# PytorchConnectomics/pytorch_connectomics

Measured on AMD Instinct MI355X. Metric: voxels/s (train + sliding-window infer), MedNeXt-S 112^3 bf16, higher is better.
Workload: dtype bf16; 1 GPU; Lucchi++ sliding-window inference (configs[1]): MedNeXt-S k3, 165x1024x768 volume, roi 112^3, overlap 0.5, bump blending, sw_batch_size 8, random-init weights; step = one whole-volume EagerSlidingWindowEngine call (TTA off); value = window-voxels/s; sw_batch_size=8, window_pipeline_streams=3

## Files before the change

### pytorch_connectomics_amd/csrc/build.py

```python
from __future__ import annotations

import hashlib
import os
import subprocess
import sys
from concurrent.futures import ThreadPoolExecutor
from pathlib import Path

CSRC = Path(__file__).resolve().parent
PKG = CSRC.parent
LIB_DIR = PKG / "lib"
LIB = LIB_DIR / "libpytc_hip.so"
ARCH = "gfx950"
FLAGS = ["-O3", "-std=c++17", "-fPIC", f"--offload-arch={ARCH}", "-Wno-unused-result"]


_NO_SLP = os.environ.get("PYTC_NO_SLP_FILES", "dwconv_kernels.hip,dwconv_mfma_kernels.hip,train_kernels.hip,rsunet_train_kernels.hip,"
                         "conv3d_strided_kernels.hip,loss_optim_kernels.hip,volume_kernels.hip,upcat_kernels.hip")
EXTRA_FLAGS = {p.name: ["-fno-slp-vectorize"] for p in Path(__file__).resolve().parent.glob("*.hip")
               if _NO_SLP == "all" or p.name in _NO_SLP.split(",")}

NO_SPILL_KERNELS = {"dwconv_kernels.hip": ("dwconv3d_k3_march_kernel", "dw_wgrad_march_kernel"),
                    "dwconv_mfma_kernels.hip": ("dwconv3d_k3_mfma_kernel",)}


def _check_no_spills(fname: str, remarks: str, patterns) -> None:
    import re
    name = None
    for line in remarks.splitlines():
        m = re.search(r"Function Name: (\S+)", line)
        if m:
            name = m.group(1)
            continue
        m = re.search(r"(VGPRs Spill|ScratchSize \[bytes/lane\]): (\d+)", line)
        if m and name and any(p in name for p in patterns) and int(m.group(2)) != 0:
            raise RuntimeError(f"{fname}: kernel {name} reports {m.group(1)} = {m.group(2)}; the asm-load / counted-wait kernels "
                               "must be spill-free (lower the occupancy hint of that instantiation)")


def asm_listing(src: Path, hipcc: str = "/opt/rocm/bin/hipcc") -> str:
    import tempfile
    with tempfile.TemporaryDirectory() as td:
        out = Path(td) / (src.stem + ".s")
        subprocess.run([hipcc, *FLAGS, *EXTRA_FLAGS.get(src.name, []), "-S", "--cuda-device-only", str(src), "-o", str(out)],
                       check=True, capture_output=True)
        return out.read_text()


def _check_asm_load_discipline(src: Path, hipcc: str) -> None:
    from . import asm_check
    text = asm_listing(src, hipcc)
    pats = NO_SPILL_KERNELS[src.name]
    if asm_check.asm_loads_in(text, pats) == 0:
        raise RuntimeError(f"{src.name}: no asm-issued register loads found in kernels {pats}: the ISA check would be checking nothing")
    bad = asm_check.check_listing(text, pats)
    if bad:
        raise RuntimeError(f"{src.name}: {len(bad)} violations of the asm-load discipline (csrc/asm_check.py), e.g.\n  " + "\n  ".join(bad[:5]))


def _check_packed_fp32_selects(obj: Path) -> None:
    import re
    objdump = Path(os.environ.get("HIPCC", "/opt/rocm/bin/hipcc")).resolve().parent.parent / "lib" / "llvm" / "bin" / "llvm-objdump"
    if not objdump.exists():
        objdump = Path("/opt/rocm/lib/llvm/bin/llvm-objdump")
    if not objdump.exists():
        return
    subprocess.run([str(objdump), "--offloading", obj.name], cwd=obj.parent, check=True, capture_output=True)
    pat = re.compile(r"v_pk_(fma|mul|add)_f32 .*op_sel:\[")
    try:
        for co in obj.parent.glob(obj.name + ".*gfx950*"):
            dis = subprocess.run([str(objdump), "-d", str(co)], check=True, capture_output=True, text=True).stdout
            hits = [ln.strip() for ln in dis.splitlines() if pat.search(ln)]
            if hits:
                raise RuntimeError(f"{obj.name}: {len(hits)} packed-fp32 instructions with a low-lane high-dword select, e.g. "
                                   f"`{hits[0]}`; add the source to PYTC_NO_SLP_FILES / EXTRA_FLAGS in csrc/build.py")
    finally:
        for extra in obj.parent.glob(obj.name + ".*"):
            extra.unlink()


def _sources():
    return sorted(CSRC.glob("*.hip"))


def _digest() -> str:
    h = hashlib.sha256()
    for p in _sources() + sorted(CSRC.glob("*.h")) + [PKG.parent / "include" / "pytc_hip.h"]:
        h.update(p.name.encode())
        h.update(p.read_bytes())
    h.update(" ".join(FLAGS).encode())
    h.update(repr(sorted(EXTRA_FLAGS.items())).encode())
    return h.hexdigest()


def build(force: bool = False, verbose: bool = True) -> Path:
    LIB_DIR.mkdir(exist_ok=True)
    obj_dir = LIB_DIR / "obj"
    obj_dir.mkdir(exist_ok=True)
    stamp = LIB_DIR / "build.sha256"
    dig = _digest()
    if not force and LIB.exists() and stamp.exists() and stamp.read_text().strip() == dig:
        build_h5(verbose=verbose)
        return LIB
    hipcc = os.environ.get("HIPCC", "/opt/rocm/bin/hipcc")

    headers = sorted(CSRC.glob("*.h")) + [PKG.parent / "include" / "pytc_hip.h", Path(__file__), CSRC / "asm_check.py"]

    def object_digest(src: Path) -> str:
        h = hashlib.sha256()
        for q in [src] + headers:
            h.update(q.name.encode())
            h.update(q.read_bytes())
        h.update(" ".join(FLAGS + EXTRA_FLAGS.get(src.name, [])).encode())
        return h.hexdigest()

    def compile_one(src: Path) -> Path:
        obj = obj_dir / (src.stem + ".o")
        ostamp = obj_dir / (src.stem + ".sha256")
        odig = object_digest(src)
        if not force and obj.exists() and ostamp.exists() and ostamp.read_text().strip() == odig:
            return obj
        cmd = [hipcc, *FLAGS, *EXTRA_FLAGS.get(src.name, []), "-c", str(src), "-o", str(obj)]
        if verbose:
            print("[build]", " ".join(cmd), flush=True)
        if src.name in NO_SPILL_KERNELS:
            out = subprocess.run(cmd + ["-Rpass-analysis=kernel-resource-usage"], check=True, capture_output=True, text=True).stderr
            _check_no_spills(src.name, out, NO_SPILL_KERNELS[src.name])
            _check_asm_load_discipline(src, hipcc)
        else:
            subprocess.run(cmd, check=True)
        _check_packed_fp32_selects(obj)
        ostamp.write_text(odig)
        return obj

    with ThreadPoolExecutor(max_workers=min(8, os.cpu_count() or 1)) as ex:
        objs = list(ex.map(compile_one, _sources()))
    cmd = [hipcc, "-shared", "-fPIC", f"--offload-arch={ARCH}", *map(str, objs), "-o", str(LIB)]
    if verbose:
        print("[build]", " ".join(cmd), flush=True)
    subprocess.run(cmd, check=True)
    stamp.write_text(dig)
    build_h5(verbose=verbose)
    return LIB


H5_LIB = LIB_DIR / "libpytc_h5.so"
H5_SRC = CSRC / "host" / "h5io.c"


def build_h5(verbose: bool = True):
    for root in (os.environ.get("HDF5_ROOT"), "/opt/conda", "/usr"):
        if root and (Path(root) / "include" / "hdf5.h").exists() and list((Path(root) / "lib").glob("libhdf5.so*")):
            break
    else:
        if verbose:
            print("[build] HDF5 headers not found: libpytc_h5.so skipped")
        return None
    if H5_LIB.exists() and H5_LIB.stat().st_mtime >= H5_SRC.stat().st_mtime:
        return H5_LIB
    LIB_DIR.mkdir(exist_ok=True)
    cmd = ["gcc", "-O2", "-fPIC", "-shared", f"-I{root}/include", str(H5_SRC), f"-L{root}/lib", "-lhdf5", "-lz", "-lpthread", "-ldl",
           f"-Wl,-rpath,{root}/lib", "-o", str(H5_LIB)]
    if verbose:
        print("[build]", " ".join(cmd), flush=True)
    subprocess.run(cmd, check=True)
    return H5_LIB


if __name__ == "__main__":
    print(build(force="--force" in sys.argv))
```

### pytorch_connectomics_amd/csrc/dwconv_mfma_kernels.hip

```cpp
#include <type_traits>

#include "dwconv_march.h"
#include "pw_common.h"

namespace pytc {

typedef short s4_t __attribute__((ext_vector_type(4)));
typedef unsigned int u32x4_t __attribute__((ext_vector_type(4)));
typedef unsigned int u32x2a4_t __attribute__((ext_vector_type(2), aligned(4)));
typedef __bf16 bf2_t __attribute__((ext_vector_type(2)));
typedef float f2_t __attribute__((ext_vector_type(2)));

constexpr int MF_TY = 8, MF_TX = 8, MF_CG = 32;
constexpr int MF_EY = MF_TY + 2, MF_EX = MF_TX + 2;
constexpr int MF_EXP = 16;
constexpr int MF_CS = MF_EY * MF_EXP + 2;
constexpr int MF_IMG = MF_CG * MF_CS;
constexpr int MF_NCHUNK = MF_EY * MF_EX * (MF_CG / 8);
constexpr int MF_CPT = 2;
constexpr int MF_TS = 32;
constexpr int MF_RS = MF_TX * MF_TS + 8;

__device__ __forceinline__ unsigned short mf_bf16_bits(float f) {
  unsigned int u = __float_as_uint(f);
  u += 0x7FFFu + ((u >> 16) & 1u);
  return (unsigned short)(u >> 16);
}
__device__ __forceinline__ float mf_bf16_float(unsigned short h) { return __uint_as_float(((unsigned int)h) << 16); }

template <int N>
__device__ __forceinline__ void mf_wait_vm() { asm volatile("s_waitcnt vmcnt(%0)" : : "n"(N) : "memory"); }


template <int N>
__device__ __forceinline__ void mf_wait_vm_upto(int n) {
  if constexpr (N > 0) {
    if (n >= N) { mf_wait_vm<N>(); return; }
    mf_wait_vm_upto<N - 1>(n);
  } else {
    mf_wait_vm<0>();
  }
}

template <int PF, bool LO, int PROBE = 0, bool STORE = true, int MIXHC = 0>
__global__ void __launch_bounds__(256, MIXHC ? 3 : 4)
dwconv3d_k3_mfma_kernel(const unsigned short* __restrict__ x, unsigned short* __restrict__ y, const float* __restrict__ w,
                        const float* __restrict__ bias, float* __restrict__ stats, DwMarch g, DwMix mx) {
  static_assert(PF == 2 || PF == 3, "two or three planes in flight");
  static_assert(MIXHC == 0 || (STORE && PF == 3), "the fused block keeps the output tile and three planes in flight");
  constexpr bool MIX = MIXHC > 0;
  __shared__ __attribute__((aligned(16))) bf16x8_t w2s[MIX ? MIXHC * 2 * 64 : 1];
  __shared__ __attribute__((aligned(16))) h8_t w3s[MIX ? 2 * MIXHC * 64 : 1];
  __shared__ __attribute__((aligned(16))) float mbias[MIX ? 32 * MIXHC + 32 : 4];
  __shared__ __attribute__((aligned(16))) unsigned short image[2][MF_IMG];
  __shared__ __attribute__((aligned(16))) unsigned short otile[STORE ? 2 : 1][STORE ? MF_TY * MF_RS : 8];
  __shared__ float wl[27 * MF_CG];
  __shared__ float red[4][2][16];

  const int tid = threadIdx.x, wave = tid >> 6, lane = tid & 63;
  int b = g.swizzle ? xcd_swizzle(blockIdx.x, gridDim.x) : blockIdx.x;
  const int ncg = g.C / MF_CG;
  const int cg = g.cg_inner ? b % ncg : (b / g.slots) % ncg;
  const int slot_id = g.cg_inner ? (b / ncg) % g.slots : b % g.slots;
  const int n = b / (ncg * g.slots);
  b = slot_id;
  const int fx = b % g.tx; b /= g.tx;
  const int fy = b % g.ty;
  const int zchunk = b / g.ty;
  const int y0 = fy * MF_TY, x0 = fx * MF_TX;
  const int zs = zchunk * g.zc;
  const int ze = min(zs + g.zc, g.D);
  const int C = g.C;
  const long plane_elems = (long)g.H * g.W * C;
  const unsigned short* xn = x + (long)n * g.D * plane_elems + cg * MF_CG;
  unsigned short* yn = y + (long)n * g.D * plane_elems + cg * MF_CG;
  const bool inner = y0 >= 1 && y0 + MF_TY + 1 <= g.H && x0 >= 1 && x0 + MF_TX + 1 <= g.W;

  for (int i = tid; i < 27 * MF_CG; i += 256) wl[i] = w[(long)(i / MF_CG) * C + cg * MF_CG + (i % MF_CG)];
  if constexpr (MIX) {
    const bf16x8_t* w2g = mx.w2n + (long)n * mx.w2_stride;
    for (int i = tid; i < MIXHC * 2 * 64; i += 256) { w2s[i] = w2g[i]; w3s[i] = mx.w3[i]; }
    if (tid < 32 * MIXHC) mbias[tid] = mx.b2n[(long)n * (32 * MIXHC) + tid];
    else if (tid < 32 * MIXHC + 32) mbias[tid] = mx.b3[tid - 32 * MIXHC];
  }
  __syncthreads();

  int goff[MF_CPT], loff[MF_CPT];
  bool cok[MF_CPT];
#pragma unroll
  for (int i = 0; i < MF_CPT; ++i) {
    const int c = tid + 256 * i;
    const int vox = c >> 2, part = c & 3;
    const int yy = vox / MF_EX, xx = vox % MF_EX;
    const int gy = y0 - 1 + yy, gx = x0 - 1 + xx;
    cok[i] = (c < MF_NCHUNK) && gy >= 0 && gy < g.H && gx >= 0 && gx < g.W;
    const int gyc = min(max(gy, 0), g.H - 1), gxc = min(max(gx, 0), g.W - 1);
    goff[i] = (gyc * g.W + gxc) * C + part * 8;
    loff[i] = (c < MF_NCHUNK) ? (part * 8) * MF_CS + yy * MF_EXP + xx : -1;
  }
  u32x4_t stg[PF][MF_CPT];
  auto issue = [&](int gz, u32x4_t (&st)[MF_CPT]) {
    const int zc = min(max(gz, 0), g.D - 1);
#pragma unroll
    for (int i = 0; i < MF_CPT; ++i) {
      const unsigned short* ptr = xn + (long)zc * plane_elems + goff[i];
      asm volatile("global_load_dwordx4 %0, %1, off" : "=&v"(st[i]) : "v"(ptr) : "memory");
    }
  };
  auto landed = [&](u32x4_t (&st)[MF_CPT], int younger) {
    mf_wait_vm_upto<2 * MF_CPT + 2>(younger);
    asm volatile("" : "+v"(st[0]), "+v"(st[1]) : : "memory");
  };
  auto commit = [&](int slot, u32x4_t (&st)[MF_CPT], int gz) {
    const bool zok = gz >= 0 && gz < g.D;
#pragma unroll
    for (int i = 0; i < MF_CPT; ++i) {
      if (loff[i] < 0) continue;
      unsigned short* dst = &image[slot][loff[i]];
      if (inner && zok) {
#pragma unroll
        for (int q = 0; q < 4; ++q) {
          dst[(2 * q) * MF_CS] = (unsigned short)(st[i][q] & 0xffffu);
          dst[(2 * q + 1) * MF_CS] = (unsigned short)(st[i][q] >> 16);
        }
      } else {
        const bool ok = zok && cok[i];
#pragma unroll
        for (int q = 0; q < 4; ++q) {
          const unsigned int dw = ok ? st[i][q] : 0u;
          dst[(2 * q) * MF_CS] = (unsigned short)(dw & 0xffffu);
          dst[(2 * q + 1) * MF_CS] = (unsigned short)(dw >> 16);
        }
      }
    }
  };

  const int h = wave & 1, ph = wave >> 1;
  const int cl = lane >> 2, j = lane & 3;
  const int ch = h * 16 + cl;
  s4_t a_hi[3][2], a_lo[3][2];
#pragma unroll
  for (int dy = 0; dy < 3; ++dy)
#pragma unroll
    for (int r = 0; r < 2; ++r) {
      s4_t vh, vl;
#pragma unroll
      for (int k = 0; k < 4; ++k) {
        const int i = j;
        const int dz = 2 - i, dx = k - r;
        float wv = 0.f;
        if (i < 3 && dx >= 0 && dx < 3) wv = wl[((dz * 3 + dy) * 3 + dx) * MF_CG + ch];
        const unsigned short hb = mf_bf16_bits(wv);
        vh[k] = (short)hb;
        vl[k] = (short)mf_bf16_bits(wv - mf_bf16_float(hb));
      }
      a_hi[dy][r] = vh;
      a_lo[dy][r] = vl;
    }
  float bv = bias ? bias[cg * MF_CG + ch] : 0.f;
  asm volatile("" : "+v"(bv));

  int boff[4];
  bool pok[4][2];
#pragma unroll
  for (int u = 0; u < 4; ++u) {
    boff[u] = ch * MF_CS + (ph * 4 + j) * MF_EXP + 2 * u;
#pragma unroll
    for (int r = 0; r < 2; ++r) pok[u][r] = (y0 + ph * 4 + j) < g.H && (x0 + 2 * u + r) < g.W;
  }
  const int op = tid >> 2, opiece = tid & 3;
  const int oy = op >> 3, ox = op & 7;
  const bool ook = (y0 + oy) < g.H && (x0 + ox) < g.W;
  const long obase = ((long)(y0 + oy) * g.W + (x0 + ox)) * C + opiece * 8;
  const int orb = oy * MF_RS + ox * MF_TS + opiece * 8;
  int ooff[4];
#pragma unroll
  for (int u = 0; u < 4; ++u) ooff[u] = (ph * 4 + j) * MF_RS + (2 * u) * MF_TS + ch;
  auto flush = [&](int zo) {
    const u32x4_t o = *reinterpret_cast<const u32x4_t*>(&otile[zo & 1][orb]);
    if (ook) *reinterpret_cast<u32x4_t*>(yn + (long)zo * plane_elems + obase) = o;
  };

  const int mr = lane & 15, mkb = lane >> 4;
  const int mp = wave * 16 + mr, my = mp >> 3, mxx = mp & 7;
  const bool mok = (y0 + my) < g.H && (x0 + mxx) < g.W;
  const long mbase = ((long)min(y0 + my, g.H - 1) * g.W + min(x0 + mxx, g.W - 1)) * C + mkb * 8;
  const int mtile = my * MF_RS + mxx * MF_TS + mkb * 8;
  u32x4_t rres[MIX ? 3 : 1];
  auto issue_res = [&](int z, u32x4_t& rr) {
    const unsigned short* ptr = xn + (long)z * plane_elems + mbase;
    asm volatile("global_load_dwordx4 %0, %1, off" : "=&v"(rr) : "v"(ptr) : "memory");
  };
  auto mix = [&](int zo, u32x4_t& rr, int younger) {
    if constexpr (MIX) {
      const bf16x8_t bact = *reinterpret_cast<const bf16x8_t*>(&otile[zo & 1][mtile]);
      f32x4_t acc2[2] = {*reinterpret_cast<const f32x4_t*>(&mbias[32 * MIXHC + mkb * 8]), *reinterpret_cast<const f32x4_t*>(&mbias[32 * MIXHC + mkb * 8 + 4])};
#pragma unroll
      for (int hc = 0; hc < MIXHC; ++hc) {
        f32x4_t acc1[2] = {*reinterpret_cast<const f32x4_t*>(&mbias[hc * 32 + mkb * 8]), *reinterpret_cast<const f32x4_t*>(&mbias[hc * 32 + mkb * 8 + 4])};
#pragma unroll
        for (int mt = 0; mt < 2; ++mt) acc1[mt] = Mma<bf16_t>::mma(w2s[(hc * 2 + mt) * 64 + lane], bact, acc1[mt]);
        float gg[8];
#pragma unroll
        for (int q = 0; q < 4; ++q) { gg[q] = acc1[0][q]; gg[4 + q] = acc1[1][q]; }
        const h8_t bhh = gelu_h8_from_f32(gg);
#pragma unroll
        for (int mo = 0; mo < 2; ++mo) acc2[mo] = __builtin_amdgcn_mfma_f32_16x16x32_f16(w3s[(mo * MIXHC + hc) * 64 + lane], bhh, acc2[mo], 0, 0, 0);
      }
      float v[8];
#pragma unroll
      for (int q = 0; q < 4; ++q) { v[q] = acc2[0][q]; v[4 + q] = acc2[1][q]; }
      if (mx.residual) {
        mf_wait_vm_upto<5>(younger);
        asm volatile("" : "+v"(rr) : : "memory");
        float rv[8];
        VecIO<bf16_t, 8>::load(reinterpret_cast<const bf16_t*>(&rr), rv);
#pragma unroll
        for (int q = 0; q < 8; ++q) v[q] += rv[q];
      }
      const long vo = (long)zo * plane_elems + mbase;
      if (mx.head_w) {
        const bf16x8_t ob = Mma<bf16_t>::from_floats(v);
        if (mx.store_y && mok) *reinterpret_cast<bf16x8_t*>(yn + vo) = ob;
        const f32x4_t hh = Mma<bf16_t>::mma(mx.head_w[lane], ob, f32x4_t{0.f, 0.f, 0.f, 0.f});
        if (mok) {
          float* hy = mx.head_y + ((long)n * g.D * g.H * g.W + (vo - mkb * 8) / C) * mx.n_head;
#pragma unroll
          for (int i = 0; i < 4; ++i)
            if (mkb * 4 + i < mx.n_head) hy[mkb * 4 + i] = hh[i] + (mx.head_b ? mx.head_b[mkb * 4 + i] : 0.f);
        }
      } else if (mok) {
        VecIO<bf16_t, 8>::store(reinterpret_cast<bf16_t*>(yn + vo), v);
      }
    }
  };

  f32x4_t acc[4][2];
#pragma unroll
  for (int u = 0; u < 4; ++u)
#pragma unroll
    for (int r = 0; r < 2; ++r) acc[u][r] = f32x4_t{bv, bv, bv, 0.f};
  float s1 = 0.f, s2 = 0.f;
  unsigned long long tk[9] = {0, 0, 0, 0, 0, 0, 0, 0, 0}, tlast = 0, tstart = 0;
  auto stamp = [&](int k) {
    if constexpr (PROBE == 4) {
      const unsigned long long now = __builtin_amdgcn_s_memtime();
      tk[k] += now - tlast;
      tlast = now;
    }
  };
  if constexpr (PROBE == 4) { tstart = __builtin_amdgcn_s_memtime(); tlast = tstart; }

  auto exists_p = [&](int z) { return z <= ze; };
  auto exists_r = [&](int z) { return MIX && mx.residual && z >= zs && z < ze; };
  auto step = [&](int gz, int slot, u32x4_t (&ld)[MF_CPT], u32x4_t (&cm)[MF_CPT], u32x4_t& rn, u32x4_t& ro) {
    if constexpr (MIX) {
      if (gz - 2 >= zs) mix(gz - 2, ro, (exists_p(gz + 1) ? MF_CPT : 0) + (exists_r(gz - 1) ? 1 : 0) + (exists_p(gz + 2) ? MF_CPT : 0));
      stamp(8);
      if (exists_r(gz)) issue_res(gz, rn);
    } else {
      if (STORE && gz - 2 >= zs && PROBE != 3) flush(gz - 2);
    }
    if (gz + PF <= ze) issue(gz + PF, ld);
    stamp(0);
    const unsigned short* img = image[slot];
#pragma unroll
    for (int dy = 0; dy < ((PROBE == 1 || PROBE == 3) ? 0 : 3); ++dy) {
      s4_t bq[4];
#pragma unroll
      for (int u = 0; u < 4; ++u) bq[u] = __builtin_bit_cast(s4_t, *reinterpret_cast<const u32x2a4_t*>(img + boff[u] + dy * MF_EXP));
#pragma unroll
      for (int u = 0; u < 4; ++u)
#pragma unroll
        for (int r = 0; r < 2; ++r) acc[u][r] = __builtin_amdgcn_mfma_f32_4x4x4bf16_1k(a_hi[dy][r], bq[u], acc[u][r], 0, 0, 0);
      if (LO) {
#pragma unroll
        for (int u = 0; u < 4; ++u)
#pragma unroll
          for (int r = 0; r < 2; ++r) acc[u][r] = __builtin_amdgcn_mfma_f32_4x4x4bf16_1k(a_lo[dy][r], bq[u], acc[u][r], 0, 0, 0);
      }
    }
    stamp(1);
    if (gz + 1 <= ze) {
      landed(cm, MF_CPT * min(PF - 1, ze - gz - 1) + (exists_r(gz - 1) ? 1 : 0) + (exists_r(gz) ? 1 : 0));
      stamp(2);
      commit(slot ^ 1, cm, gz + 1);
      stamp(3);
    } else {
      mf_wait_vm<0>();
    }
    if (gz - 1 >= zs && PROBE != 3) {
      unsigned short* ot = otile[STORE ? (gz - 1) & 1 : 0];
#pragma unroll
      for (int u = 0; u < 4; ++u) {
        const bf2_t hb = __builtin_convertvector(f2_t{acc[u][0][0], acc[u][1][0]}, bf2_t);
        const unsigned int bits = __builtin_bit_cast(unsigned int, hb);
        if constexpr (STORE) {
          ot[ooff[u]] = (unsigned short)(bits & 0xffffu);
          ot[ooff[u] + MF_TS] = (unsigned short)(bits >> 16);
        }
        if constexpr (!MIX) {
          float r0 = __uint_as_float(bits << 16), r1 = __uint_as_float(bits & 0xffff0000u);
          if (!inner) { r0 = pok[u][0] ? r0 : 0.f; r1 = pok[u][1] ? r1 : 0.f; }
          s1 += r0; s2 = fmaf(r0, r0, s2);
          s1 += r1; s2 = fmaf(r1, r1, s2);
        }
      }
    }
#pragma unroll
    for (int u = 0; u < 4; ++u)
#pragma unroll
      for (int r = 0; r < 2; ++r) acc[u][r] = f32x4_t{acc[u][r][1], acc[u][r][2], bv, 0.f};
    stamp(4);
    __syncthreads();
    stamp(5);
    if constexpr (PROBE == 4) tk[6] += 1;
  };

#pragma unroll
  for (int q = 0; q < PF; ++q) issue(zs - 1 + q, stg[q]);
  landed(stg[0], MF_CPT * (PF - 1));
  commit(0, stg[0], zs - 1);
  __syncthreads();
  int slot = 0;
  for (int gz = zs - 1; gz <= ze; gz += PF) {
#pragma unroll
    for (int k = 0; k < PF; ++k) {
      if (gz + k <= ze) { step(gz + k, slot, stg[k], stg[(k + 1) % PF], rres[MIX ? k : 0], rres[MIX ? (k + 1) % 3 : 0]); slot ^= 1; }
    }
  }
  mf_wait_vm<0>();
  if constexpr (MIX) {
    const int rs = (ze - zs) % 3;
    if (rs == 0) mix(ze - 1, rres[0], 0);
    else if (rs == 1) mix(ze - 1, rres[MIX ? 1 : 0], 0);
    else mix(ze - 1, rres[MIX ? 2 : 0], 0);
  } else {
    if (STORE && PROBE != 3) flush(ze - 1);
  }

  if constexpr (PROBE == 4) {
    if constexpr (MIX) {
      if (mx.prof && lane == 0) {
        tk[7] = __builtin_amdgcn_s_memtime() - tstart;
        float* o = mx.prof + (((long)n * g.slots + slot_id) * 4 + wave) * 9;
#pragma unroll
        for (int k = 0; k < 9; ++k) o[k] = (float)tk[k];
      }
    } else if (stats && lane == 0) {
      tk[7] = __builtin_amdgcn_s_memtime() - tstart;
      float* o = stats + (((long)n * g.slots + slot_id) * 2) * C + cg * MF_CG + wave * 8;
#pragma unroll
      for (int k = 0; k < 8; ++k) o[k] = (float)tk[k];
    }
    return;
  }
  if (!MIX && stats) {
    s1 += __shfl_xor(s1, 1, 64); s2 += __shfl_xor(s2, 1, 64);
    s1 += __shfl_xor(s1, 2, 64); s2 += __shfl_xor(s2, 2, 64);
    if (j == 0) { red[wave][0][cl] = s1; red[wave][1][cl] = s2; }
    __syncthreads();
    if (tid < 2 * MF_CG) {
      const int which = tid / MF_CG, chn = tid % MF_CG;
      const float a = red[chn >> 4][which][chn & 15] + red[(chn >> 4) + 2][which][chn & 15];
      stats[(((long)n * g.slots + slot_id) * 2 + which) * C + cg * MF_CG + chn] = a;
    }
  }
}

void dwconv_mfma_launch(const void* x, void* y, const float* w, const float* bias, float* stats, const DwMarch& g, int variant,
                        hipStream_t s) {
  dim3 grid((unsigned)((long)g.slots * (g.C / MF_CG) * g.N)), block(256);
  const unsigned short* xp = (const unsigned short*)x;
  unsigned short* yp = (unsigned short*)y;
  const DwMix none{};
#define PYTC_MF(PFV, LOV, NM) hipLaunchKernelGGL((dwconv3d_k3_mfma_kernel<PFV, LOV, NM>), grid, block, 0, s, xp, yp, w, bias, stats, g, none)
#define PYTC_MF_STATS(PFV, LOV) hipLaunchKernelGGL((dwconv3d_k3_mfma_kernel<PFV, LOV, 0, false>), grid, block, 0, s, xp, yp, w, bias, stats, g, none)
  const int probe = tuning_get("dwconv_mfma_probe", 0);
  if (!y) {
    if (variant & 1) { if (variant & 2) PYTC_MF_STATS(2, true); else PYTC_MF_STATS(3, true); }
    else { if (variant & 2) PYTC_MF_STATS(2, false); else PYTC_MF_STATS(3, false); }
  }
  else if (probe == 1) PYTC_MF(3, false, 1);
  else if (probe == 3) PYTC_MF(3, false, 3);
  else if (probe == 4) PYTC_MF(3, false, 4);
  else if (variant & 1) { if (variant & 2) PYTC_MF(2, true, 0); else PYTC_MF(3, true, 0); }
  else { if (variant & 2) PYTC_MF(2, false, 0); else PYTC_MF(3, false, 0); }
#undef PYTC_MF
#undef PYTC_MF_STATS
}

int dwmix_launch(const void* x, void* y, const float* w, const float* bias, const DwMarch& g, const DwMix& mx, int c_hid, int variant,
                 hipStream_t s) {
  dim3 grid((unsigned)((long)g.slots * g.N)), block(256);
  const unsigned short* xp = (const unsigned short*)x;
  unsigned short* yp = (unsigned short*)y;
#define PYTC_DM(LOV, HCV, PRB) hipLaunchKernelGGL((dwconv3d_k3_mfma_kernel<3, LOV, PRB, true, HCV>), grid, block, 0, s, xp, yp, w, bias, (float*)nullptr, g, mx)
  const bool lo = variant & 1;
  if (mx.prof) {
    if (c_hid != 64 || lo) return -1;
    PYTC_DM(false, 2, 4);
    return 0;
  }
  switch (c_hid) {
    case 64: if (lo) PYTC_DM(true, 2, 0); else PYTC_DM(false, 2, 0); break;
    case 96: if (lo) PYTC_DM(true, 3, 0); else PYTC_DM(false, 3, 0); break;
    case 128: if (lo) PYTC_DM(true, 4, 0); else PYTC_DM(false, 4, 0); break;
    default: return -1;
  }
#undef PYTC_DM
  return 0;
}

}
```

Measured before the change: 1.820 billion voxels/s.

## Add warp-specialized fused dwconv+MLP kernel with separate conv and mix waves

Adds a 512-thread kernel where four waves run the depthwise 3x3x3 MFMA march and four other waves run the pointwise expand/GELU/project mix (plus residual and optional head) on the previous plane via a double-buffered LDS output tile. It becomes the default path for the fused dwmix launch through an env/tuning switch. The intent is to overlap the depthwise convolution and the channel-mixing matmuls instead of running them serially in one set of waves. The cost is more LDS per block, 2 blocks per CU rather than 3, and barrier coupling between the two wave groups.

```diff
diff --git a/pytorch_connectomics_amd/csrc/build.py b/pytorch_connectomics_amd/csrc/build.py
--- a/pytorch_connectomics_amd/csrc/build.py
+++ b/pytorch_connectomics_amd/csrc/build.py
@@ -21,7 +21,7 @@
                if _NO_SLP == "all" or p.name in _NO_SLP.split(",")}
 
 NO_SPILL_KERNELS = {"dwconv_kernels.hip": ("dwconv3d_k3_march_kernel", "dw_wgrad_march_kernel"),
-                    "dwconv_mfma_kernels.hip": ("dwconv3d_k3_mfma_kernel",)}
+                    "dwconv_mfma_kernels.hip": ("dwconv3d_k3_mfma_kernel", "dwmix_waves_kernel")}
 
 
 def _check_no_spills(fname: str, remarks: str, patterns) -> None:
diff --git a/pytorch_connectomics_amd/csrc/dwconv_mfma_kernels.hip b/pytorch_connectomics_amd/csrc/dwconv_mfma_kernels.hip
--- a/pytorch_connectomics_amd/csrc/dwconv_mfma_kernels.hip
+++ b/pytorch_connectomics_amd/csrc/dwconv_mfma_kernels.hip
@@ -1,3 +1,5 @@
+#include <stdlib.h>
+
 #include <type_traits>
 
 #include "dwconv_march.h"
@@ -31,6 +33,8 @@
 template <int N>
 __device__ __forceinline__ void mf_wait_vm() { asm volatile("s_waitcnt vmcnt(%0)" : : "n"(N) : "memory"); }
 
+
+__device__ __forceinline__ void mf_lds_barrier() { asm volatile("s_waitcnt lgkmcnt(0)\n\ts_barrier" : : : "memory"); }
 
 template <int N>
 __device__ __forceinline__ void mf_wait_vm_upto(int n) {
@@ -368,6 +372,273 @@
   }
 }
 
+template <bool LO, int MIXHC>
+__global__ void __launch_bounds__(512, 2)
+dwmix_waves_kernel(const unsigned short* __restrict__ x, unsigned short* __restrict__ y, const float* __restrict__ w,
+                   const float* __restrict__ bias, DwMarch g, DwMix mx) {
+  constexpr int PF = 3;
+  __shared__ __attribute__((aligned(16))) bf16x8_t w2s[MIXHC * 2 * 64];
+  __shared__ __attribute__((aligned(16))) h8_t w3s[2 * MIXHC * 64];
+  __shared__ __attribute__((aligned(16))) float mbias[32 * MIXHC + 32];
+  __shared__ __attribute__((aligned(16))) unsigned short image[2][MF_IMG];
+  __shared__ __attribute__((aligned(16))) unsigned short otile[2][MF_TY * MF_RS];
+  __shared__ float wl[27 * MF_CG];
+
+  const int tid = threadIdx.x, lane = tid & 63;
+  const int wave = __builtin_amdgcn_readfirstlane(tid >> 6);
+  int b = g.swizzle ? xcd_swizzle(blockIdx.x, gridDim.x) : blockIdx.x;
+  const int slot_id = b % g.slots;
+  const int n = b / g.slots;
+  b = slot_id;
+  const int fx = b % g.tx; b /= g.tx;
+  const int fy = b % g.ty;
+  const int zchunk = b / g.ty;
+  const int y0 = fy * MF_TY, x0 = fx * MF_TX;
+  const int zs = zchunk * g.zc;
+  const int ze = min(zs + g.zc, g.D);
+  const int C = MF_CG;
+  const long plane_elems = (long)g.H * g.W * C;
+  const unsigned short* xn = x + (long)n * g.D * plane_elems;
+  unsigned short* yn = y + (long)n * g.D * plane_elems;
+
+  for (int i = tid; i < 27 * MF_CG; i += 512) wl[i] = w[i];
+  {
+    const bf16x8_t* w2g = mx.w2n + (long)n * mx.w2_stride;
+    for (int i = tid; i < MIXHC * 2 * 64; i += 512) { w2s[i] = w2g[i]; w3s[i] = mx.w3[i]; }
+    if (tid < 32 * MIXHC) mbias[tid] = mx.b2n[(long)n * (32 * MIXHC) + tid];
+    else if (tid < 32 * MIXHC + 32) mbias[tid] = mx.b3[tid - 32 * MIXHC];
+  }
+  __syncthreads();
+
+  if (wave < 4) {
+    const bool inner = y0 >= 1 && y0 + MF_TY + 1 <= g.H && x0 >= 1 && x0 + MF_TX + 1 <= g.W;
+    int goff[MF_CPT], loff[MF_CPT];
+    bool cok[MF_CPT];
+#pragma unroll
+    for (int i = 0; i < MF_CPT; ++i) {
+      const int c = tid + 256 * i;
+      const int vox = c >> 2, part = c & 3;
+      const int yy = vox / MF_EX, xx = vox % MF_EX;
+      const int gy = y0 - 1 + yy, gx = x0 - 1 + xx;
+      cok[i] = (c < MF_NCHUNK) && gy >= 0 && gy < g.H && gx >= 0 && gx < g.W;
+      const int gyc = min(max(gy, 0), g.H - 1), gxc = min(max(gx, 0), g.W - 1);
+      goff[i] = (gyc * g.W + gxc) * C + part * 8;
+      loff[i] = (c < MF_NCHUNK) ? (part * 8) * MF_CS + yy * MF_EXP + xx : -1;
+    }
+    u32x4_t stg[PF][MF_CPT];
+    auto issue = [&](int gz, u32x4_t (&st)[MF_CPT]) {
+      const int zc = min(max(gz, 0), g.D - 1);
+#pragma unroll
+      for (int i = 0; i < MF_CPT; ++i) {
+        const unsigned short* ptr = xn + (long)zc * plane_elems + goff[i];
+        asm volatile("global_load_dwordx4 %0, %1, off" : "=&v"(st[i]) : "v"(ptr) : "memory");
+      }
+    };
+    auto landed = [&](u32x4_t (&st)[MF_CPT], int younger) {
+      mf_wait_vm_upto<2 * MF_CPT>(younger);
+      asm volatile("" : "+v"(st[0]), "+v"(st[1]) : : "memory");
+    };
+    auto commit = [&](int slot, u32x4_t (&st)[MF_CPT], int gz) {
+      const bool zok = gz >= 0 && gz < g.D;
+#pragma unroll
+      for (int i = 0; i < MF_CPT; ++i) {
+        if (loff[i] < 0) continue;
+        unsigned short* dst = &image[slot][loff[i]];
+        if (inner && zok) {
+#pragma unroll
+          for (int q = 0; q < 4; ++q) {
+            dst[(2 * q) * MF_CS] = (unsigned short)(st[i][q] & 0xffffu);
+            dst[(2 * q + 1) * MF_CS] = (unsigned short)(st[i][q] >> 16);
+          }
+        } else {
+          const bool ok = zok && cok[i];
+#pragma unroll
+          for (int q = 0; q < 4; ++q) {
+            const unsigned int dw = ok ? st[i][q] : 0u;
+            dst[(2 * q) * MF_CS] = (unsigned short)(dw & 0xffffu);
+            dst[(2 * q + 1) * MF_CS] = (unsigned short)(dw >> 16);
+          }
+        }
+      }
+    };
+
+    const int h = wave & 1, ph = wave >> 1;
+    const int cl = lane >> 2, j = lane & 3;
+    const int ch = h * 16 + cl;
+    s4_t a_hi[3][2], a_lo[3][2];
+#pragma unroll
+    for (int dy = 0; dy < 3; ++dy)
+#pragma unroll
+      for (int r = 0; r < 2; ++r) {
+        s4_t vh, vl;
+#pragma unroll
+        for (int k = 0; k < 4; ++k) {
+          const int i = j;
+          const int dz = 2 - i, dx = k - r;
+          float wv = 0.f;
+          if (i < 3 && dx >= 0 && dx < 3) wv = wl[((dz * 3 + dy) * 3 + dx) * MF_CG + ch];
+          const unsigned short hb = mf_bf16_bits(wv);
+          vh[k] = (short)hb;
+          vl[k] = (short)mf_bf16_bits(wv - mf_bf16_float(hb));
+        }
+        a_hi[dy][r] = vh;
+        a_lo[dy][r] = vl;
+      }
+    float bv = bias ? bias[ch] : 0.f;
+    asm volatile("" : "+v"(bv));
+
+    int boff[4], ooff[4];
+#pragma unroll
+    for (int u = 0; u < 4; ++u) {
+      boff[u] = ch * MF_CS + (ph * 4 + j) * MF_EXP + 2 * u;
+      ooff[u] = (ph * 4 + j) * MF_RS + (2 * u) * MF_TS + ch;
+    }
+    f32x4_t acc[4][2];
+#pragma unroll
+    for (int u = 0; u < 4; ++u)
+#pragma unroll
+      for (int r = 0; r < 2; ++r) acc[u][r] = f32x4_t{bv, bv, bv, 0.f};
+
+    auto step = [&](int gz, int slot, u32x4_t (&ld)[MF_CPT], u32x4_t (&cm)[MF_CPT]) {
+      if (gz + PF <= ze) issue(gz + PF, ld);
+      const unsigned short* img = image[slot];
+#pragma unroll
+      for (int dy = 0; dy < 3; ++dy) {
+        s4_t bq[4];
+#pragma unroll
+        for (int u = 0; u < 4; ++u) bq[u] = __builtin_bit_cast(s4_t, *reinterpret_cast<const u32x2a4_t*>(img + boff[u] + dy * MF_EXP));
+#pragma unroll
+        for (int u = 0; u < 4; ++u)
+#pragma unroll
+          for (int r = 0; r < 2; ++r) acc[u][r] = __builtin_amdgcn_mfma_f32_4x4x4bf16_1k(a_hi[dy][r], bq[u], acc[u][r], 0, 0, 0);
+        if (LO) {
+#pragma unroll
+          for (int u = 0; u < 4; ++u)
+#pragma unroll
+            for (int r = 0; r < 2; ++r) acc[u][r] = __builtin_amdgcn_mfma_f32_4x4x4bf16_1k(a_lo[dy][r], bq[u], acc[u][r], 0, 0, 0);
+        }
+      }
+      if (gz + 1 <= ze) {
+        landed(cm, MF_CPT * min(PF - 1, ze - gz - 1));
+        commit(slot ^ 1, cm, gz + 1);
+      } else {
+        mf_wait_vm<0>();
+      }
+      if (gz - 1 >= zs) {
+        unsigned short* ot = otile[(gz - 1) & 1];
+#pragma unroll
+        for (int u = 0; u < 4; ++u) {
+          const bf2_t hb = __builtin_convertvector(f2_t{acc[u][0][0], acc[u][1][0]}, bf2_t);
+          const unsigned int bits = __builtin_bit_cast(unsigned int, hb);
+          ot[ooff[u]] = (unsigned short)(bits & 0xffffu);
+          ot[ooff[u] + MF_TS] = (unsigned short)(bits >> 16);
+        }
+      }
+#pragma unroll
+      for (int u = 0; u < 4; ++u)
+#pragma unroll
+        for (int r = 0; r < 2; ++r) acc[u][r] = f32x4_t{acc[u][r][1], acc[u][r][2], bv, 0.f};
+      __syncthreads();
+    };
+
+#pragma unroll
+    for (int q = 0; q < PF; ++q) issue(zs - 1 + q, stg[q]);
+    landed(stg[0], MF_CPT * (PF - 1));
+    commit(0, stg[0], zs - 1);
+    __syncthreads();
+    int slot = 0;
+    for (int gz = zs - 1; gz <= ze; gz += PF) {
+#pragma unroll
+      for (int k = 0; k < PF; ++k) {
+        if (gz + k <= ze) { step(gz + k, slot, stg[k], stg[(k + 1) % PF]); slot ^= 1; }
+      }
+    }
+    mf_wait_vm<0>();
+  } else {
+    const int mr = lane & 15, mkb = lane >> 4;
+    const int mp = (wave - 4) * 16 + mr, my = mp >> 3, mxx = mp & 7;
+    const bool mok = (y0 + my) < g.H && (x0 + mxx) < g.W;
+    const long mbase = ((long)min(y0 + my, g.H - 1) * g.W + min(x0 + mxx, g.W - 1)) * C + mkb * 8;
+    const int mtile = my * MF_RS + mxx * MF_TS + mkb * 8;
+    bf16x8_t hw{};
+    float hb[4] = {0.f, 0.f, 0.f, 0.f};
+    if (mx.head_w) {
+      hw = mx.head_w[lane];
+#pragma unroll
+      for (int i = 0; i < 4; ++i)
+        if (mx.head_b && mkb * 4 + i < mx.n_head) hb[i] = mx.head_b[mkb * 4 + i];
+    }
+    auto issue_res = [&](int z, u32x4_t& rr) {
+      const unsigned short* ptr = xn + (long)z * plane_elems + mbase;
+      asm volatile("global_load_dwordx4 %0, %1, off" : "=&v"(rr) : "v"(ptr) : "memory");
+    };
+    auto mix = [&](int zo, u32x4_t& rr, int younger, auto res_tag) {
+      constexpr bool RES = decltype(res_tag)::value;
+      const bf16x8_t bact = *reinterpret_cast<const bf16x8_t*>(&otile[zo & 1][mtile]);
+      f32x4_t acc2[2] = {*reinterpret_cast<const f32x4_t*>(&mbias[32 * MIXHC + mkb * 8]), *reinterpret_cast<const f32x4_t*>(&mbias[32 * MIXHC + mkb * 8 + 4])};
+#pragma unroll
+      for (int hc = 0; hc < MIXHC; ++hc) {
+        f32x4_t acc1[2] = {*reinterpret_cast<const f32x4_t*>(&mbias[hc * 32 + mkb * 8]), *reinterpret_cast<const f32x4_t*>(&mbias[hc * 32 + mkb * 8 + 4])};
+#pragma unroll
+        for (int mt = 0; mt < 2; ++mt) acc1[mt] = Mma<bf16_t>::mma(w2s[(hc * 2 + mt) * 64 + lane], bact, acc1[mt]);
+        float gg[8];
+#pragma unroll
+        for (int q = 0; q < 4; ++q) { gg[q] = acc1[0][q]; gg[4 + q] = acc1[1][q]; }
+        const h8_t bhh = gelu_h8_from_f32(gg);
+#pragma unroll
+        for (int mo = 0; mo < 2; ++mo) acc2[mo] = __builtin_amdgcn_mfma_f32_16x16x32_f16(w3s[(mo * MIXHC + hc) * 64 + lane], bhh, acc2[mo], 0, 0, 0);
+      }
+      float v[8];
+#pragma unroll
+      for (int q = 0; q < 4; ++q) { v[q] = acc2[0][q]; v[4 + q] = acc2[1][q]; }
+      if constexpr (RES) {
+        mf_wait_vm_upto<1>(younger);
+        asm volatile("" : "+v"(rr) : : "memory");
+        float rv[8];
+        VecIO<bf16_t, 8>::load(reinterpret_cast<const bf16_t*>(&rr), rv);
+#pragma unroll
+        for (int q = 0; q < 8; ++q) v[q] += rv[q];
+      }
+      const long vo = (long)zo * plane_elems + mbase;
+      if (mx.head_w) {
+        const bf16x8_t ob = Mma<bf16_t>::from_floats(v);
+        if (mx.store_y && mok) *reinterpret_cast<bf16x8_t*>(yn + vo) = ob;
+        const f32x4_t hh = Mma<bf16_t>::mma(hw, ob, f32x4_t{0.f, 0.f, 0.f, 0.f});
+        if (mok) {
+          float* hy = mx.head_y + ((long)n * g.D * g.H * g.W + (vo - mkb * 8) / C) * mx.n_head;
+#pragma unroll
+          for (int i = 0; i < 4; ++i)
+            if (mkb * 4 + i < mx.n_head) hy[mkb * 4 + i] = hh[i] + hb[i];
+        }
+      } else if (mok) {
+        VecIO<bf16_t, 8>::store(reinterpret_cast<bf16_t*>(yn + vo), v);
+      }
+    };
+    auto march = [&](auto res_tag) {
+      constexpr bool RES = decltype(res_tag)::value;
+      u32x4_t rres[2] = {u32x4_t{0u, 0u, 0u, 0u}, u32x4_t{0u, 0u, 0u, 0u}};
+      mf_lds_barrier();
+      for (int gz0 = zs - 1; gz0 <= ze; gz0 += 2) {
+#pragma unroll
+        for (int k = 0; k < 2; ++k) {
+          const int gz = gz0 + k;
+          if (gz <= ze) {
+            if (gz - 2 >= zs) mix(gz - 2, rres[k], gz - 1 < ze ? 1 : 0, res_tag);
+            else if (RES) mf_wait_vm<1>();
+            if (RES && gz >= zs && gz < ze) issue_res(gz, rres[k]);
+            mf_lds_barrier();
+          }
+        }
+      }
+      mf_wait_vm<0>();
+      u32x4_t rlast = ((ze - zs) & 1) ? rres[1] : rres[0];
+      mix(ze - 1, rlast, 0, res_tag);
+    };
+    if (mx.residual) march(std::true_type{});
+    else march(std::false_type{});
+  }
+}
+
 void dwconv_mfma_launch(const void* x, void* y, const float* w, const float* bias, float* stats, const DwMarch& g, int variant,
                         hipStream_t s) {
   dim3 grid((unsigned)((long)g.slots * (g.C / MF_CG) * g.N)), block(256);
@@ -397,6 +668,19 @@
   unsigned short* yp = (unsigned short*)y;
 #define PYTC_DM(LOV, HCV, PRB) hipLaunchKernelGGL((dwconv3d_k3_mfma_kernel<3, LOV, PRB, true, HCV>), grid, block, 0, s, xp, yp, w, bias, (float*)nullptr, g, mx)
   const bool lo = variant & 1;
+  static const int waves_env = [] { const char* e = getenv("PYTC_DWMIX_WAVES"); return e ? atoi(e) : 1; }();
+  if (!mx.prof && tuning_get("dwmix_waves", waves_env) != 0) {
+    const dim3 wblock(512);
+#define PYTC_DW(LOV, HCV) hipLaunchKernelGGL((dwmix_waves_kernel<LOV, HCV>), grid, wblock, 0, s, xp, yp, w, bias, g, mx)
+    switch (c_hid) {
+      case 64: if (lo) PYTC_DW(true, 2); else PYTC_DW(false, 2); break;
+      case 96: if (lo) PYTC_DW(true, 3); else PYTC_DW(false, 3); break;
+      case 128: if (lo) PYTC_DW(true, 4); else PYTC_DW(false, 4); break;
+      default: return -1;
+    }
+#undef PYTC_DW
+    return 0;
+  }
   if (mx.prof) {
     if (c_hid != 64 || lo) return -1;
     PYTC_DM(false, 2, 4);
```

Result: no change. 1.820 billion voxels/s (median of 6 runs) (+0.0%).
